# annihilatorrrr/spacedrive

Hardware: AMD Instinct MI355X
Metric: cas_ids/sec + hashed GB/s (whole node), 10M files at 1/2/4/8 MI355X (higher is better)
Workload: dtype u32; 1 GPU; sampled-path cas_id (57,352-B BLAKE3 message/file) + Object grouping; 1310720 files/GPU/step (1310720 per step at n_gpus=1); dup_permille=300, parallelism=shard-by-file x1, grouping=fused

## Files before the change

include/sd_hip_cas.h:

```cpp
#ifndef SD_HIP_CAS_H
#define SD_HIP_CAS_H

#include <stddef.h>
#include <stdint.h>

#ifdef __cplusplus
extern "C" {
#endif

#define SD_CAS_ABI_VERSION 1

#define SD_CAS_SAMPLE_COUNT 4u
#define SD_CAS_SAMPLE_SIZE (1024u * 10u)
#define SD_CAS_HEADER_OR_FOOTER_SIZE (1024u * 8u)
#define SD_CAS_MINIMUM_FILE_SIZE (1024u * 100u)
#define SD_CAS_SAMPLED_CONTENT_LEN (2u * SD_CAS_HEADER_OR_FOOTER_SIZE + SD_CAS_SAMPLE_COUNT * SD_CAS_SAMPLE_SIZE)
#define SD_CAS_CHUNK_SIZE 100u
#define SD_CAS_MAX_PACKED_CONTENT_LEN (104u * 1024u - 8u)

#define SD_CAS_OK 0
#define SD_CAS_EINVAL (-1)
#define SD_CAS_EHIP (-2)
#define SD_CAS_EIO (-3)
#define SD_CAS_ENOMEM (-4)
// ... 50 lines not shown
                               const char* prefix, uint32_t stride, char* d_out, void* stream);

int sd_cas_hash_sampled_dev(sd_cas_ctx* ctx, const void* d_content, uint64_t stride,
                            const uint64_t* d_sizes, size_t n, uint64_t* d_keys, void* stream);

int sd_cas_hash_packed_dev(sd_cas_ctx* ctx, const void* d_arena, const uint64_t* d_offs,
                           const uint32_t* d_lens, const uint64_t* d_sizes, size_t n,
                           uint64_t* d_keys, void* stream);

int sd_cas_group_dev(sd_cas_ctx* ctx, const uint64_t* d_keys, size_t n, uint32_t* d_rep,
                     uint64_t* out_objects, void* stream);
int sd_cas_hash_group_sampled_dev(sd_cas_ctx* ctx, const void* d_content, uint64_t stride,
                                  const uint64_t* d_sizes, size_t n, uint64_t* d_keys,
                                  uint32_t* d_rep, uint32_t* d_overflow, uint64_t* out_objects,
                                  void* stream);
int sd_cas_hash_regions_sampled_dev(sd_cas_ctx* ctx, const void* d_content, uint64_t stride,
                                    const uint64_t* d_sizes, size_t n, uint64_t* d_keys,
                                    uint32_t* d_rep, uint32_t* d_overflow, void* stream);
int sd_cas_group_regions_dev(sd_cas_ctx* ctx, size_t n, uint32_t* d_rep, uint64_t* out_objects,
                             void* stream);
int sd_cas_set_dup_verify(sd_cas_ctx* ctx, int on);
int sd_cas_dup_verify_counters(sd_cas_ctx* ctx, uint64_t* out_candidates, uint64_t* out_verified,
                               uint64_t* out_rehashed);
int sd_cas_group_min_dev(sd_cas_ctx* ctx, const uint64_t* d_keys, const uint32_t* d_vals, size_t n,
                         uint32_t* d_out, uint64_t* out_objects, void* stream);
int sd_cas_partition_dev(sd_cas_ctx* ctx, const uint64_t* d_keys, size_t n, uint32_t parts,
                         uint64_t* d_keys_out, uint32_t* d_pos_out, uint64_t* d_counts,
                         void* stream);
int sd_cas_exchange_pack_dev(sd_cas_ctx* ctx, const uint64_t* d_keys, const uint32_t* d_pos,
                             size_t n, uint64_t file0, uint32_t* d_rows, void* stream);
int sd_cas_exchange_split_dev(sd_cas_ctx* ctx, const uint32_t* d_rows, size_t m,
                              uint64_t* d_keys, uint32_t* d_vals, void* stream);
int sd_cas_exchange_unpack_dev(sd_cas_ctx* ctx, const uint32_t* d_back, const uint32_t* d_pos,
                               size_t n, uint64_t* d_rep, void* stream);
int sd_cas_exchange_pack_fixed_dev(sd_cas_ctx* ctx, const uint64_t* d_keys, const uint32_t* d_pos,
                                   const uint64_t* d_counts, uint32_t G, uint64_t cap,
                                   uint64_t spill, uint64_t file0, uint32_t* d_rows,
                                   uint32_t* d_spill_rows, uint32_t* d_overflow, void* stream);
int sd_cas_exchange_split_fixed_dev(sd_cas_ctx* ctx, const uint32_t* d_rows, size_t m,
                                    uint64_t sentinel, uint64_t* d_keys, uint32_t* d_vals,
                                    uint64_t* d_sentinel_rows, void* stream);
int sd_cas_exchange_unpack_fixed_dev(sd_cas_ctx* ctx, const uint32_t* d_back,
                                     const uint32_t* d_spill_back, const uint32_t* d_pos,
                                     const uint64_t* d_counts, uint32_t G, uint64_t cap,
                                     uint64_t spill, uint64_t* d_rep, void* stream);
int sd_cas_copy_objects_dev(sd_cas_ctx* ctx, uint64_t* d_dst, void* stream);
// ... 125 lines not shown
```

rust/sd-hip-cas/src/lib.rs:

```rust
#![allow(non_camel_case_types)]
use std::{
    ffi::{c_char, c_int, c_void, CStr, CString},
    io,
    os::unix::ffi::OsStrExt,
    path::{Path, PathBuf},
    ptr,
};

#[repr(C)]
pub struct sd_cas_ctx {
    _p: [u8; 0],
}

#[repr(C)]
pub struct sd_cas_multi {
    _p: [u8; 0],
}

pub const SD_CAS_ROW_HASHED: u8 = 0;
pub const SD_CAS_ROW_NO_CAS: u8 = 1;
pub const SD_CAS_ROW_ERROR: u8 = 2;
pub const SD_CAS_LINK_CREATED: u8 = 0;
pub const SD_CAS_LINK_LINKED: u8 = 1;
pub const SD_CAS_LINK_DROPPED: u8 = 2;
// ... 52 lines not shown
                                      prefix: *const c_char, stride: u32, d_out: *mut c_char,
                                      stream: *mut c_void) -> c_int;
    pub fn sd_cas_hash_sampled_dev(ctx: *mut sd_cas_ctx, d_content: *const c_void, stride: u64,
                                   d_sizes: *const u64, n: usize, d_keys: *mut u64,
                                   stream: *mut c_void) -> c_int;
    pub fn sd_cas_hash_packed_dev(ctx: *mut sd_cas_ctx, d_arena: *const c_void, d_offs: *const u64,
                                  d_lens: *const u32, d_sizes: *const u64, n: usize, d_keys: *mut u64,
                                  stream: *mut c_void) -> c_int;
    pub fn sd_cas_group_dev(ctx: *mut sd_cas_ctx, d_keys: *const u64, n: usize, d_rep: *mut u32,
                            out_objects: *mut u64, stream: *mut c_void) -> c_int;
    pub fn sd_cas_hash_group_sampled_dev(ctx: *mut sd_cas_ctx, d_content: *const c_void, stride: u64,
                                         d_sizes: *const u64, n: usize, d_keys: *mut u64,
                                         d_rep: *mut u32, d_overflow: *mut u32,
                                         out_objects: *mut u64, stream: *mut c_void) -> c_int;
    pub fn sd_cas_hash_regions_sampled_dev(ctx: *mut sd_cas_ctx, d_content: *const c_void, stride: u64,
                                           d_sizes: *const u64, n: usize, d_keys: *mut u64,
                                           d_rep: *mut u32, d_overflow: *mut u32,
                                           stream: *mut c_void) -> c_int;
    pub fn sd_cas_group_regions_dev(ctx: *mut sd_cas_ctx, n: usize, d_rep: *mut u32,
                                    out_objects: *mut u64, stream: *mut c_void) -> c_int;
    pub fn sd_cas_set_dup_verify(ctx: *mut sd_cas_ctx, on: c_int) -> c_int;
    pub fn sd_cas_dup_verify_counters(ctx: *mut sd_cas_ctx, out_candidates: *mut u64,
                                      out_verified: *mut u64, out_rehashed: *mut u64) -> c_int;
    pub fn sd_cas_group_min_dev(ctx: *mut sd_cas_ctx, d_keys: *const u64, d_vals: *const u32, n: usize,
                                d_out: *mut u32, out_objects: *mut u64, stream: *mut c_void) -> c_int;
    pub fn sd_cas_partition_dev(ctx: *mut sd_cas_ctx, d_keys: *const u64, n: usize, parts: u32,
                                d_keys_out: *mut u64, d_pos_out: *mut u32, d_counts: *mut u64,
                                stream: *mut c_void) -> c_int;
    pub fn sd_cas_exchange_pack_dev(ctx: *mut sd_cas_ctx, d_keys: *const u64, d_pos: *const u32,
                                    n: usize, file0: u64, d_rows: *mut u32, stream: *mut c_void) -> c_int;
    pub fn sd_cas_exchange_split_dev(ctx: *mut sd_cas_ctx, d_rows: *const u32, m: usize,
                                     d_keys: *mut u64, d_vals: *mut u32, stream: *mut c_void) -> c_int;
    pub fn sd_cas_exchange_unpack_dev(ctx: *mut sd_cas_ctx, d_back: *const u32, d_pos: *const u32,
                                      n: usize, d_rep: *mut u64, stream: *mut c_void) -> c_int;
    pub fn sd_cas_exchange_pack_fixed_dev(ctx: *mut sd_cas_ctx, d_keys: *const u64, d_pos: *const u32,
                                          d_counts: *const u64, G: u32, cap: u64, spill: u64,
                                          file0: u64, d_rows: *mut u32, d_spill_rows: *mut u32,
                                          d_overflow: *mut u32, stream: *mut c_void) -> c_int;
    pub fn sd_cas_exchange_split_fixed_dev(ctx: *mut sd_cas_ctx, d_rows: *const u32, m: usize,
                                           sentinel: u64, d_keys: *mut u64, d_vals: *mut u32,
                                           d_sentinel_rows: *mut u64, stream: *mut c_void) -> c_int;
    pub fn sd_cas_exchange_unpack_fixed_dev(ctx: *mut sd_cas_ctx, d_back: *const u32,
                                            d_spill_back: *const u32, d_pos: *const u32,
                                            d_counts: *const u64, G: u32, cap: u64, spill: u64,
                                            d_rep: *mut u64, stream: *mut c_void) -> c_int;
    pub fn sd_cas_copy_objects_dev(ctx: *mut sd_cas_ctx, d_dst: *mut u64, stream: *mut c_void) -> c_int;
// ... 508 lines not shown
```

spacedrive_amd/_native.py:

```python
from __future__ import annotations

import ctypes
import os
import subprocess

HERE = os.path.dirname(os.path.abspath(__file__))
LIB_PATH = os.environ.get("SD_HIP_CAS_LIB") or os.path.join(HERE, "libsd_hip_cas.so")
CSRC = os.path.join(HERE, "csrc")

SD_CAS_OK = 0
ERRORS = {-1: "EINVAL", -2: "EHIP", -3: "EIO", -4: "ENOMEM", -5: "ENODEV"}

_vp, _sz, _u64, _u32, _i = ctypes.c_void_p, ctypes.c_size_t, ctypes.c_uint64, ctypes.c_uint32, ctypes.c_int
_cp = ctypes.c_char_p
SIGNATURES = [
    ("sd_cas_abi_version", _i, []),
    ("sd_cas_ctx_create", _i, [_i, ctypes.POINTER(_vp)]),
    ("sd_cas_ctx_destroy", None, [_vp]),
    ("sd_cas_last_error", _cp, [_vp]),
    ("sd_cas_ctx_stream", _vp, [_vp]),
    ("sd_cas_synchronize", _i, [_vp]),
    ("sd_cas_batch_quantum", _sz, [_vp]),
    ("sd_cas_set_latency_threshold", None, [_vp, _sz, _sz]),
    ("sd_cas_set_chunkpar_split", None, [_vp, _sz, _sz]),
    ("sd_cas_set_group_method", _i, [_vp, _i, _u64]),
    ("sd_cas_alloc_pinned", _i, [_vp, _sz, ctypes.POINTER(_vp)]),
    ("sd_cas_free_pinned", _i, [_vp, _vp]),
    ("sd_cas_generate_cas_ids", _i, [_vp, _vp, _vp, _vp, _sz, _vp]),
    ("sd_cas_generate_cas_ids_from_paths", _i, [_vp, _vp, _vp, _sz, _vp, _vp]),
    ("sd_cas_file_metadata_from_paths", _i, [_vp, _vp, _sz, _vp, _vp, _vp]),
    ("sd_cas_hash_sampled_host", _i, [_vp, _vp, _u64, _vp, _sz, _vp, _sz]),
    ("sd_cas_hash_sampled_host_ring", _i, [_vp, _vp, _u64, _sz, _vp, _sz, _vp, _sz]),
    ("sd_cas_key_to_hex", None, [_u64, _cp]),
    ("sd_cas_shard_hex", None, [_u64, _cp]),
    ("sd_cas_thumbnail_path", ctypes.c_int64, [_cp, _cp, _u64, _cp, _sz]),
    ("sd_cas_thumb_key", ctypes.c_int64, [_cp, _u64, _cp, _sz]),
    ("sd_cas_keys_to_hex_dev", _i, [_vp, _vp, _sz, _vp, _vp]),
    ("sd_cas_thumbnail_paths_dev", _i, [_vp, _vp, _sz, _cp, _u32, _vp, _vp]),
    ("sd_cas_hash_sampled_dev", _i, [_vp, _vp, _u64, _vp, _sz, _vp, _vp]),
    ("sd_cas_hash_packed_dev", _i, [_vp, _vp, _vp, _vp, _vp, _sz, _vp, _vp]),
    ("sd_cas_group_dev", _i, [_vp, _vp, _sz, _vp, _vp, _vp]),
    ("sd_cas_hash_group_sampled_dev", _i, [_vp, _vp, _u64, _vp, _sz, _vp, _vp, _vp, _vp, _vp]),
    ("sd_cas_hash_regions_sampled_dev", _i, [_vp, _vp, _u64, _vp, _sz, _vp, _vp, _vp, _vp]),
    ("sd_cas_group_regions_dev", _i, [_vp, _sz, _vp, _vp, _vp]),
    ("sd_cas_set_dup_verify", _i, [_vp, _i]),
    ("sd_cas_dup_verify_counters", _i, [_vp, _vp, _vp, _vp]),
    ("sd_cas_group_min_dev", _i, [_vp, _vp, _vp, _sz, _vp, _vp, _vp]),
    ("sd_cas_partition_dev", _i, [_vp, _vp, _sz, _u32, _vp, _vp, _vp, _vp]),
    ("sd_cas_exchange_pack_dev", _i, [_vp, _vp, _vp, _sz, _u64, _vp, _vp]),
    ("sd_cas_exchange_split_dev", _i, [_vp, _vp, _sz, _vp, _vp, _vp]),
    ("sd_cas_exchange_unpack_dev", _i, [_vp, _vp, _vp, _sz, _vp, _vp]),
    ("sd_cas_exchange_pack_fixed_dev", _i, [_vp, _vp, _vp, _vp, _u32, _u64, _u64, _u64, _vp, _vp, _vp, _vp]),
    ("sd_cas_exchange_split_fixed_dev", _i, [_vp, _vp, _sz, _u64, _vp, _vp, _vp, _vp]),
    ("sd_cas_exchange_unpack_fixed_dev", _i, [_vp, _vp, _vp, _vp, _vp, _u32, _u64, _u64, _vp, _vp]),
    ("sd_cas_copy_objects_dev", _i, [_vp, _vp, _vp]),
    ("sd_cas_group_sorted_dev", _i, [_vp, _vp, _vp, _sz, _vp, _vp, _vp]),
    ("sd_cas_group_chunked_dev", _i, [_vp, _vp, _sz, _u32, _vp, _vp, _vp, _vp]),
    ("sd_cas_identifier_max_steps", _sz, [_sz, _u32]),
    ("sd_cas_identifier_links_dev", _i, [_vp, _vp, _vp, _sz, _u32, _vp, _vp, _vp, _vp, _sz, _vp, _vp]),
    ("sd_cas_identifier_links", _i, [_vp, _vp, _vp, _sz, _u32, _vp, _vp, _vp, _vp, _sz, _vp]),
    ("sd_cas_identifier_links_seeded_dev", _i,
     [_vp, _vp, _vp, _sz, _u32, _vp, _vp, _sz, _vp, _vp, _vp, _vp, _sz, _vp, _vp]),
    ("sd_cas_identifier_links_seeded", _i,
     [_vp, _vp, _vp, _sz, _u32, _vp, _vp, _sz, _vp, _vp, _vp, _vp, _sz, _vp]),
    ("sd_cas_identifier_links_ex_dev", _i,
     [_vp, _vp, _vp, _sz, _u32, _vp, _vp, _sz, _vp, _vp, _vp, _vp, _vp, _sz, _vp, _vp]),
    ("sd_cas_identifier_links_ex", _i,
     [_vp, _vp, _vp, _sz, _u32, _vp, _vp, _sz, _vp, _vp, _vp, _vp, _vp, _sz, _vp]),
    ("sd_cas_object_stats_dev", _i, [_vp, _vp, _vp, _sz, _vp, _vp, _vp, _vp]),
# ... 63 lines not shown
```

spacedrive_amd/cas.py:

```python
from __future__ import annotations

import ctypes
import os
from dataclasses import dataclass, field
from typing import Optional, Sequence

import numpy as np

from . import _native
from ._native import CasError

SAMPLE_COUNT = 4
SAMPLE_SIZE = 1024 * 10
HEADER_OR_FOOTER_SIZE = 1024 * 8
MINIMUM_FILE_SIZE = 1024 * 100
SAMPLED_CONTENT_LEN = 2 * HEADER_OR_FOOTER_SIZE + SAMPLE_COUNT * SAMPLE_SIZE
CHUNK_SIZE = 100
MAX_PACKED_CONTENT_LEN = 104 * 1024 - 8
THRESHOLD_DEFAULT = (1 << 64) - 1
NO_OBJECT = NO_STEP = 0xFFFFFFFF
STAT_NAMES = ("rows", "objects", "total_bytes", "unique_bytes", "duplicate_sets", "max_copies",
              "size_mismatch_rows", "bad_rows")
TOP_MAX = 65536
TOP_TILE = 16384
# ... 290 lines not shown
                             stream: Optional[int] = None) -> None:
        n = int(sizes.numel())
        stride = int(content.shape[-1]) if content.dim() == 2 else SAMPLED_CONTENT_LEN
        self._check(self.L.sd_cas_hash_regions_sampled_dev(
            self.h, _ptr(content), stride, _ptr(sizes), n, _ptr(keys), _ptr(rep), _ptr(overflow),
            _stream(stream)), "hash_regions_sampled")

    def group_regions(self, n: int, rep, stream: Optional[int] = None,
                      want_objects: bool = True) -> Optional[int]:
        obj = ctypes.c_uint64(0)
        self._check(self.L.sd_cas_group_regions_dev(self.h, int(n), _ptr(rep),
                                                    ctypes.byref(obj) if want_objects else None,
                                                    _stream(stream)), "group_regions")
        return int(obj.value) if want_objects else None

    def set_dup_verify(self, on: bool = True) -> None:
        self._check(self.L.sd_cas_set_dup_verify(self.h, 1 if on else 0), "set_dup_verify")

    def dup_verify_counters(self) -> tuple[int, int, int]:
        c, v, r = ctypes.c_uint64(0), ctypes.c_uint64(0), ctypes.c_uint64(0)
        self._check(self.L.sd_cas_dup_verify_counters(self.h, ctypes.byref(c), ctypes.byref(v),
                                                      ctypes.byref(r)), "dup_verify_counters")
        return int(c.value), int(v.value), int(r.value)

    def group_min(self, keys, vals, out, stream: Optional[int] = None,
                  want_objects: bool = True) -> Optional[int]:
        n = int(keys.numel())
        obj = ctypes.c_uint64(0)
        self._check(self.L.sd_cas_group_min_dev(
            self.h, _ptr(keys), _ptr(vals) if vals is not None else None, n, _ptr(out),
            ctypes.byref(obj) if want_objects else None, _stream(stream)), "group_min")
        return int(obj.value) if want_objects else None

    def exchange_pack(self, keys, pos, file0: int, rows, stream: Optional[int] = None) -> None:
        self._check(self.L.sd_cas_exchange_pack_dev(self.h, _ptr(keys), _ptr(pos), int(keys.numel()),
                                                    int(file0), _ptr(rows), _stream(stream)),
                    "exchange_pack")

    def exchange_split(self, rows, keys, vals, stream: Optional[int] = None) -> None:
        self._check(self.L.sd_cas_exchange_split_dev(self.h, _ptr(rows), int(keys.numel()), _ptr(keys),
                                                     _ptr(vals), _stream(stream)), "exchange_split")

    def exchange_unpack(self, back, pos, rep, stream: Optional[int] = None) -> None:
        self._check(self.L.sd_cas_exchange_unpack_dev(self.h, _ptr(back), _ptr(pos), int(back.numel()),
                                                      _ptr(rep), _stream(stream)), "exchange_unpack")

# ... 388 lines not shown
```

spacedrive_amd/csrc/cas_hash.hip:

```cpp
#include <hip/hip_runtime.h>
#include <stdint.h>

#include "blake3_lane.hpp"
#include "blake3_tree.hpp"
#include "sd_dup_probe.h"
#include "sd_group.h"
#include "sd_kernels.h"
#include "sd_mix.h"
#include "sd_ws.h"

namespace sdcas {


constexpr uint32_t SAMPLED_PAIRS = SAMPLED_CONTENT_LEN / 128;
constexpr uint32_t SAMPLED_CHUNKS = SAMPLED_CONTENT_LEN / 1024;
static_assert(SAMPLED_PAIRS == 8 * SAMPLED_CHUNKS, "the sampled content is whole chunks of 8 lines");

__device__ __forceinline__ void load_pair_here(const uint4* __restrict__ q, uint32_t P,
                                               uint4 (&buf)[8]) {
  __builtin_amdgcn_sched_barrier(0);
  line(q, P, buf);
  __builtin_amdgcn_sched_barrier(0);
}

constexpr int SAMPLED_DEPTH = 5;
constexpr int SAMPLED_BLOCK = 512;

template <int B = SAMPLED_BLOCK>
// ... 150 lines not shown
  if (blockIdx.x == 0 && threadIdx.x < 2) ro.objects[threadIdx.x] = 0;
  region_epilogue<B>(stack_lds, live, f, key, keys, ro);
}

extern "C" __global__ void __launch_bounds__(SAMPLED_BLOCK)
sd_cas_sampled_group_kernel(const uint8_t* __restrict__ content, uint64_t stride,
                            const uint64_t* __restrict__ sizes, uint64_t n,
                            uint64_t* __restrict__ keys, RegionOut ro) {
  sampled_group_kernel_body<SAMPLED_BLOCK>(content, stride, sizes, n, keys, ro);
}

extern "C" __global__ void __launch_bounds__(SAMPLED_BLOCK_NARROW)
sd_cas_sampled_group_kernel_256(const uint8_t* __restrict__ content, uint64_t stride,
                                const uint64_t* __restrict__ sizes, uint64_t n,
                                uint64_t* __restrict__ keys, RegionOut ro) {
  sampled_group_kernel_body<SAMPLED_BLOCK_NARROW>(content, stride, sizes, n, keys, ro);
}

struct DupLists {
  const uint32_t* cand;
  uint32_t* list_h;
  uint32_t* list_c;
  uint32_t* same;
  uint32_t* counters;
  uint32_t tail_tiles;
  volatile uint32_t* note;
  uint32_t seq, files;
};
constexpr uint32_t DUP_N_HASH = 0, DUP_N_CAND = 1, DUP_VERIFIED = 2, DUP_REHASHED = 3, DUP_QUEUE = 4;

extern "C" __global__ void __launch_bounds__(256)
sd_dup_probe_kernel(const uint8_t* __restrict__ content, uint64_t stride,
                    const uint64_t* __restrict__ sizes, uint64_t n, uint64_t* __restrict__ probes,
                    uint32_t* __restrict__ counters) {
  const uint64_t f = (uint64_t)blockIdx.x * 256 + threadIdx.x;
  if (blockIdx.x == 0 && threadIdx.x < DUP_COUNTERS) counters[threadIdx.x] = 0;
  if (f < n) probes[f] = dup_probe(sizes[f], content + f * stride);
}

extern "C" __global__ void __launch_bounds__(256)
sd_dup_compact_kernel(uint64_t n, DupLists dl) {
  __shared__ uint32_t wcnt[2][4], base[2];
  const uint64_t f = (uint64_t)blockIdx.x * 256 + threadIdx.x;
  const uint32_t lane = threadIdx.x & 63u, w = threadIdx.x >> 6;
  const bool live = f < n;
  const bool h = live && dl.cand[f] == (uint32_t)f;
  const bool c = live && !h;
  const uint64_t bh = __ballot(h), bc = __ballot(c);
  const uint64_t below = (1ull << lane) - 1ull;
  if (lane == 0) {
    wcnt[0][w] = (uint32_t)__popcll(bh);
    wcnt[1][w] = (uint32_t)__popcll(bc);
  }
  __syncthreads();
  if (threadIdx.x < 2) {
    const uint32_t t = wcnt[threadIdx.x][0] + wcnt[threadIdx.x][1] + wcnt[threadIdx.x][2] +
                       wcnt[threadIdx.x][3];
    base[threadIdx.x] = t ? atomicAdd(&dl.counters[threadIdx.x ? DUP_N_CAND : DUP_N_HASH], t) : 0u;
  }
  __syncthreads();
  uint32_t oh = base[0] + (uint32_t)__popcll(bh & below);
  uint32_t oc = base[1] + (uint32_t)__popcll(bc & below);
  for (uint32_t i = 0; i < w; ++i) {
    oh += wcnt[0][i];
    oc += wcnt[1][i];
  }
  if (h) dl.list_h[oh] = (uint32_t)f;
  if (c) dl.list_c[oc] = (uint32_t)f;
}

constexpr uint32_t CMP_QUADS = SAMPLED_CONTENT_LEN / 16;
constexpr uint32_t CMP_UNROLL = 8;
static_assert(CMP_QUADS % (64 * CMP_UNROLL) == 0, "a row is whole compare rounds");
__device__ __forceinline__ bool rows_equal(const uint4* __restrict__ a, const uint4* __restrict__ b,
                                           uint32_t lane) {
#pragma unroll 1
  for (uint32_t q = lane; q < CMP_QUADS; q += 64 * CMP_UNROLL) {
    uint4 x[CMP_UNROLL], y[CMP_UNROLL];
#pragma unroll
    for (uint32_t u = 0; u < CMP_UNROLL; ++u) x[u] = a[q + 64 * u];
#pragma unroll
    for (uint32_t u = 0; u < CMP_UNROLL; ++u) y[u] = b[q + 64 * u];
    uint32_t d = 0;
#pragma unroll
    for (uint32_t u = 0; u < CMP_UNROLL; ++u)
      d |= (x[u].x ^ y[u].x) | (x[u].y ^ y[u].y) | (x[u].z ^ y[u].z) | (x[u].w ^ y[u].w);
    if (__ballot(d != 0)) return false;
  }
  return true;
}

template <int B>
__device__ __forceinline__ void dup_mixed_kernel_body(const uint8_t* __restrict__ content,
                                                      uint64_t stride,
                                                      const uint64_t* __restrict__ sizes,
                                                      uint64_t* __restrict__ keys, RegionOut ro,
                                                      DupLists dl) {
  __shared__ uint32_t stack_lds[SAMPLED_DEPTH][8][B];
  const uint32_t n_hash = dl.counters[DUP_N_HASH], n_cand = dl.counters[DUP_N_CAND];
  const uint32_t G = gridDim.x;
  const uint32_t TH = (n_hash + B - 1) / B;
  const uint32_t TC = G - TH;
  const uint32_t TT = TC < dl.tail_tiles ? TC : dl.tail_tiles;
  const uint32_t GI = G - TT, TI = TC - TT;
  const bool tail = blockIdx.x >= GI;
  const uint32_t c0 = tail ? 0u : (uint32_t)((uint64_t)blockIdx.x * TI / GI);
  const uint32_t c1 = tail ? 1u : (uint32_t)(((uint64_t)blockIdx.x + 1) * TI / GI);
  if (blockIdx.x == 0 && threadIdx.x < 2) ro.objects[threadIdx.x] = 0;
  if (blockIdx.x == 0 && threadIdx.x == 0 && dl.note) {
    dl.note[1] = n_cand;
    dl.note[2] = dl.files;
    __threadfence_system();
    dl.note[0] = dl.seq;
  }
  if (c0 == c1) {
    const uint32_t i = (blockIdx.x - c0) * B + threadIdx.x;
    const bool live = i < n_hash;
    uint64_t f = 0, key = 0;
    if (live) {
      f = dl.list_h[i];
      LdsStack<B> stk{stack_lds, threadIdx.x};
      const uint4* q = reinterpret_cast<const uint4*>(content + f * stride);
      key = cas_lane_sampled<B>(q, sizes[f], stk);
    }
    region_epilogue<B>(stack_lds, live, f, key, keys, ro);
  } else {
    const uint32_t lane = threadIdx.x & 63u;
    for (uint32_t k = 0; tail || k < 64u; ++k) {
      uint32_t p = 0;
      if (lane == 0) p = atomicAdd(&dl.counters[DUP_QUEUE], 1u);
      p = __builtin_amdgcn_readfirstlane(p);
      if (p >= n_cand) break;
      const uint32_t f = dl.list_c[p], g = dl.cand[f];
      bool eq = sizes[f] == sizes[g];
      if (eq)
        eq = rows_equal(reinterpret_cast<const uint4*>(content + (uint64_t)f * stride),
                        reinterpret_cast<const uint4*>(content + (uint64_t)g * stride), lane);
      if (lane == 0) dl.same[f] = eq ? 1u : 0u;
    }
  }
}

extern "C" __global__ void __launch_bounds__(SAMPLED_BLOCK)
sd_cas_dup_mixed_kernel(const uint8_t* __restrict__ content, uint64_t stride,
                        const uint64_t* __restrict__ sizes, uint64_t* __restrict__ keys,
                        RegionOut ro, DupLists dl) {
  dup_mixed_kernel_body<SAMPLED_BLOCK>(content, stride, sizes, keys, ro, dl);
}

extern "C" __global__ void __launch_bounds__(SAMPLED_BLOCK_NARROW)
sd_cas_dup_mixed_kernel_256(const uint8_t* __restrict__ content, uint64_t stride,
                            const uint64_t* __restrict__ sizes, uint64_t* __restrict__ keys,
                            RegionOut ro, DupLists dl) {
  dup_mixed_kernel_body<SAMPLED_BLOCK_NARROW>(content, stride, sizes, keys, ro, dl);
}

extern "C" __global__ void __launch_bounds__(SAMPLED_BLOCK_NARROW)
sd_cas_dup_finish_kernel(const uint8_t* __restrict__ content, uint64_t stride,
                         const uint64_t* __restrict__ sizes, uint64_t* __restrict__ keys,
                         RegionOut ro, DupLists dl) {
  constexpr int B = SAMPLED_BLOCK_NARROW;
// ... 163 lines not shown
                                uint32_t* rfile, uint32_t* cursor, uint64_t cap, uint64_t* spill_keys,
                                uint32_t* spill_file, uint32_t* overflow, uint64_t* objects,
                                hipStream_t s, uint32_t cus) {
  if (n == 0) return hipSuccess;
  const RegionOut ro{rkeys, rfile, cursor, cap, spill_keys, spill_file, rep, overflow,
                     (unsigned long long*)objects};
  const uint64_t blocks = (n + SAMPLED_BLOCK - 1) / SAMPLED_BLOCK;
  const uint64_t quanta = cus ? (n + (uint64_t)cus * 256 - 1) / ((uint64_t)cus * 256) : 0;
  if (cus && (blocks < cus || (quanta & 1))) {
    const uint64_t nb = (n + SAMPLED_BLOCK_NARROW - 1) / SAMPLED_BLOCK_NARROW;
    sd_cas_sampled_group_kernel_256<<<(uint32_t)nb, SAMPLED_BLOCK_NARROW, 0, s>>>(content, stride,
                                                                                 sizes, n, keys, ro);
  } else {
    sd_cas_sampled_group_kernel<<<(uint32_t)blocks, SAMPLED_BLOCK, 0, s>>>(content, stride, sizes, n,
                                                                          keys, ro);
  }
  return hipGetLastError();
}

DupVerifyWs dup_verify_layout(void* ws, uint64_t n) {
  WsCarve w(ws);  DupVerifyWs L;
  L.probes = w.take<uint64_t>(n);  L.cand = w.take<uint32_t>(n);
  L.list_h = w.take<uint32_t>(n);  L.list_c = w.take<uint32_t>(n);  L.same = w.take<uint32_t>(n);
  L.counters = w.take<uint32_t>(DUP_COUNTERS);  L.objects = w.take<uint64_t>(1);
  L.bytes = w.bytes();  return L;
}
size_t dup_verify_workspace_bytes(uint64_t n) { return dup_verify_layout(nullptr, n).bytes; }

hipError_t dup_candidates(const uint8_t* content, uint64_t stride, const uint64_t* sizes, uint64_t n,
                          const DupVerifyWs& L, void* group_ws, uint32_t* totals, hipStream_t s) {
  if (n == 0) return hipSuccess;
  sd_dup_probe_kernel<<<(uint32_t)((n + 255) / 256), 256, 0, s>>>(content, stride, sizes, n, L.probes,
                                                                  L.counters);
  hipError_t e = hipGetLastError();
  if (e != hipSuccess) return e;
  return hash_group_min(L.probes, nullptr, n, L.cand, L.objects, group_ws, totals, s);
}

hipError_t hash_sampled_regions_verify(const uint8_t* content, uint64_t stride, const uint64_t* sizes,
                                       uint64_t n, uint64_t* keys, uint32_t* rep, uint64_t* rkeys,
                                       uint32_t* rfile, uint32_t* cursor, uint64_t cap,
                                       uint64_t* spill_keys, uint32_t* spill_file, uint32_t* overflow,
                                       uint64_t* objects, const DupVerifyWs& L, uint32_t* note,
                                       uint32_t seq, hipStream_t s, uint32_t cus) {
  if (n == 0) return hipSuccess;
  const RegionOut ro{rkeys, rfile, cursor, cap, spill_keys, spill_file, rep, overflow,
                     (unsigned long long*)objects};
  const uint64_t blocks = (n + SAMPLED_BLOCK - 1) / SAMPLED_BLOCK;
  const uint64_t quanta = cus ? (n + (uint64_t)cus * 256 - 1) / ((uint64_t)cus * 256) : 0;
  const bool narrow = cus && (blocks < cus || (quanta & 1));
  const uint32_t slots = (cus ? cus : 256u) * (narrow ? 4u : 2u);
  const uint32_t tail_tiles = slots * 5u / 7u;
  const DupLists dl{L.cand, L.list_h, L.list_c, L.same, L.counters, tail_tiles, note, seq, (uint32_t)n};
  sd_dup_compact_kernel<<<(uint32_t)((n + 255) / 256), 256, 0, s>>>(n, dl);
  if (narrow) {
    const uint64_t nb = (n + SAMPLED_BLOCK_NARROW - 1) / SAMPLED_BLOCK_NARROW;
    sd_cas_dup_mixed_kernel_256<<<(uint32_t)nb + 1, SAMPLED_BLOCK_NARROW, 0, s>>>(content, stride, sizes,
                                                                                 keys, ro, dl);
  } else {
    sd_cas_dup_mixed_kernel<<<(uint32_t)blocks + 1, SAMPLED_BLOCK, 0, s>>>(content, stride, sizes, keys,
                                                                          ro, dl);
  }
  const uint64_t fb = (n + SAMPLED_BLOCK_NARROW - 1) / SAMPLED_BLOCK_NARROW;
  sd_cas_dup_finish_kernel<<<(uint32_t)fb, SAMPLED_BLOCK_NARROW, 0, s>>>(content, stride, sizes, keys,
                                                                        ro, dl);
  return hipGetLastError();
}

#ifndef SD_PULL_UNROLL
#define SD_PULL_UNROLL 4
#endif
#ifndef SD_PULL_WIDE_BYTES
#define SD_PULL_WIDE_BYTES (512u << 10)
#endif
template <int U>
__global__ void __launch_bounds__(256)
sd_pull_host(const uint4* __restrict__ src, uint4* __restrict__ dst, uint64_t quads) {
// ... 59 lines not shown
```

spacedrive_amd/csrc/sd_hip_cas.cpp:

```cpp
#include <ctype.h>
#include <errno.h>
#include <fcntl.h>
#include <hip/hip_runtime.h>
#include <stdarg.h>
#include <stdio.h>
#include <stdlib.h>
#include <string.h>
#include <sys/stat.h>
#include <unistd.h>

#include <algorithm>
#include <atomic>
#include <memory>
#include <string>
#include <thread>
#include <vector>

#include "sd_checksum.h"
#include "sd_group.h"
#include "sd_kernels.h"
#include "sd_links.h"
#include "sd_mix.h"
#include "sd_object_stats.h"
#include "sd_synth.h"
// ... 527 lines not shown
      e = hash_sampled_regions_verify((const uint8_t*)d_content, stride, d_sizes, n, d_keys, d_rep,
                                      L.rkeys, L.rfile, cur, region_capacity(n), L.spill_keys,
                                      L.spill_file, d_overflow, L.objects, D, c->dupv_note,
                                      ++c->dupv_seq, s, (uint32_t)(c->quantum / 256));
    c->dupv_n = e == hipSuccess ? n : 0;
    c->dupv_stream = s;
  } else {
    e = hash_sampled_regions((const uint8_t*)d_content, stride, d_sizes, n, d_keys, d_rep,
                             L.rkeys, L.rfile, cur, region_capacity(n), L.spill_keys,
                             L.spill_file, d_overflow, L.objects, s, (uint32_t)(c->quantum / 256));
    c->dupv_n = 0;
  }
  if (e != hipSuccess) {
    (void)hipMemsetAsync(cur, 0, REGION_SET_WORDS * 4, s);
    return fail(c, SD_CAS_EHIP, "hash_regions: %s", hipGetErrorString(e));
  }
  HIP_TRY(c, hipEventRecord(c->region_hashed[k], s));
  c->region_keys[k] = d_keys;
  c->region_cur = k;
  c->region_grouped[k] = false;
  return SD_CAS_OK;
}

int sd_cas_dup_verify_counters(sd_cas_ctx* c, uint64_t* out_candidates, uint64_t* out_verified,
                               uint64_t* out_rehashed) {
  if (!c || !out_candidates || !out_verified || !out_rehashed) return SD_CAS_EINVAL;
  uint32_t h[DUP_COUNTERS] = {0};
  if (c->dupv_n && c->region_cur >= 0) {
    HIP_TRY(c, hipSetDevice(c->device));
    HIP_TRY(c, hipStreamWaitEvent(c->stream, c->region_hashed[c->region_cur], 0));
    HIP_TRY(c, hipMemcpyAsync(h, dup_verify_layout(c->dupv.p, c->dupv_n).counters, sizeof h,
                              hipMemcpyDeviceToHost, c->stream));
    HIP_TRY(c, hipStreamSynchronize(c->stream));
  }
  *out_candidates = h[1];
  *out_verified = h[2];
  *out_rehashed = h[3];
  return SD_CAS_OK;
}

int sd_cas_group_regions_dev(sd_cas_ctx* c, size_t n, uint32_t* d_rep, uint64_t* out_objects,
                             void* stream) {
  if (!c) return SD_CAS_EINVAL;
  const int k = c->region_cur;
  if (k < 0 || c->region_grouped[k] || c->region_n[k] != n || !d_rep)
    return fail(c, SD_CAS_EINVAL, "group_regions: no ungrouped hash_regions batch of %zu files", n);
  HIP_TRY(c, hipSetDevice(c->device));
  hipStream_t s = pick(c, stream);
  const RegionGroupWs L = region_group_layout(c->regions[k].p, c->region_n[k]);
  uint32_t* cur = c->gcursor + REGION_SET_WORDS * k;
  HIP_TRY(c, hipStreamWaitEvent(s, c->region_hashed[k], 0));
  hipError_t e = region_group_min(L.rkeys, L.rfile, cur, region_capacity(n), d_rep, L.objects, L.gkeys, L.gvals,
                                  c->region_keys[k], n, L.spill_keys, L.spill_file, c->test_table_fill, s);
  if (e != hipSuccess) {
    (void)hipMemsetAsync(cur, 0, REGION_SET_WORDS * 4, s);
    return fail(c, SD_CAS_EHIP, "group_regions: %s", hipGetErrorString(e));
  }
  HIP_TRY(c, hipEventRecord(c->region_done[k], s));
  c->region_pending[k] = true;
  c->region_grouped[k] = true;
// ... 590 lines not shown
```

spacedrive_amd/csrc/sd_kernels.h:

```cpp
#pragma once
#include <stdint.h>

namespace sdcas {

constexpr uint64_t SAMPLE_COUNT = 4;
constexpr uint64_t SAMPLE_SIZE = 1024 * 10;
constexpr uint64_t HEADER_OR_FOOTER_SIZE = 1024 * 8;
constexpr uint64_t MINIMUM_FILE_SIZE = 1024 * 100;
constexpr uint32_t SAMPLED_CONTENT_LEN =
    (uint32_t)(2 * HEADER_OR_FOOTER_SIZE + SAMPLE_COUNT * SAMPLE_SIZE);
static_assert(2 * HEADER_OR_FOOTER_SIZE + SAMPLE_COUNT * SAMPLE_SIZE < MINIMUM_FILE_SIZE, "cas.rs:18");
static_assert(SAMPLE_SIZE > HEADER_OR_FOOTER_SIZE, "cas.rs:21");

constexpr uint32_t MAX_PACKED_CONTENT_LEN = 104u * 1024u - 8u;

}

#include <hip/hip_runtime.h>
namespace sdcas {
hipError_t hash_sampled(const uint8_t* content, uint64_t stride, const uint64_t* sizes,
                        uint64_t n, uint64_t* keys, hipStream_t s, uint32_t cus);
hipError_t hash_sampled_regions(const uint8_t* content, uint64_t stride, const uint64_t* sizes,
                                uint64_t n, uint64_t* keys, uint32_t* rep, uint64_t* rkeys,
                                uint32_t* rfile, uint32_t* cursor, uint64_t cap, uint64_t* spill_keys,
                                uint32_t* spill_file, uint32_t* overflow, uint64_t* objects,
                                hipStream_t s, uint32_t cus);
constexpr uint32_t DUP_COUNTERS = 8;
struct DupVerifyWs {
  uint64_t* probes; uint32_t *cand, *list_h, *list_c, *same, *counters; uint64_t* objects; size_t bytes;
};
DupVerifyWs dup_verify_layout(void* ws, uint64_t n);
size_t dup_verify_workspace_bytes(uint64_t n);
hipError_t dup_candidates(const uint8_t* content, uint64_t stride, const uint64_t* sizes, uint64_t n,
                          const DupVerifyWs& L, void* group_ws, uint32_t* totals, hipStream_t s);
hipError_t hash_sampled_regions_verify(const uint8_t* content, uint64_t stride, const uint64_t* sizes,
                                       uint64_t n, uint64_t* keys, uint32_t* rep, uint64_t* rkeys,
                                       uint32_t* rfile, uint32_t* cursor, uint64_t cap,
                                       uint64_t* spill_keys, uint32_t* spill_file, uint32_t* overflow,
                                       uint64_t* objects, const DupVerifyWs& L, uint32_t* note,
                                       uint32_t seq, hipStream_t s, uint32_t cus);
hipError_t pull_host(void* dst, const void* src, uint64_t bytes, hipStream_t s);
hipError_t hash_packed(const uint8_t* arena, const uint64_t* offs, const uint32_t* lens,
                       const uint64_t* sizes, const uint32_t* order, uint64_t n, uint64_t* keys,
                       hipStream_t s);
hipError_t length_keys(const uint32_t* lens, uint64_t n, uint64_t* out, hipStream_t s);
hipError_t hash_chunkpar(const uint8_t* arena, const uint64_t* offs, uint64_t stride,
                         const uint32_t* lens, uint32_t fixed_len, const uint64_t* sizes,
                         uint64_t n, uint64_t* keys, int seg, hipStream_t s,
                         const uint32_t* order = nullptr);
int length_key_bits(uint64_t n);
struct InplaceWs { uint32_t *counters, *lens32, *sampled_idx; size_t bytes; };
InplaceWs inplace_layout(void* ws, uint64_t n);
// ... 8 lines not shown
```

Baseline: 60.72 million cas_ids/s.

## Batch duplicate verification into grouped runs sharing reference slice loads

After: 61.62 million cas_ids/s (median of 6 runs). 1.5% higher.

```diff
diff --git a/include/sd_hip_cas.h b/include/sd_hip_cas.h
--- a/include/sd_hip_cas.h
+++ b/include/sd_hip_cas.h
@@ -96,6 +96,8 @@
 int sd_cas_set_dup_verify(sd_cas_ctx* ctx, int on);
 int sd_cas_dup_verify_counters(sd_cas_ctx* ctx, uint64_t* out_candidates, uint64_t* out_verified,
                                uint64_t* out_rehashed);
+int sd_cas_dup_verify_rows(sd_cas_ctx* ctx, uint64_t* out_groups, uint64_t* out_tasks,
+                           uint64_t* out_references);
 int sd_cas_group_min_dev(sd_cas_ctx* ctx, const uint64_t* d_keys, const uint32_t* d_vals, size_t n,
                          uint32_t* d_out, uint64_t* out_objects, void* stream);
 int sd_cas_partition_dev(sd_cas_ctx* ctx, const uint64_t* d_keys, size_t n, uint32_t parts,
diff --git a/rust/sd-hip-cas/src/lib.rs b/rust/sd-hip-cas/src/lib.rs
--- a/rust/sd-hip-cas/src/lib.rs
+++ b/rust/sd-hip-cas/src/lib.rs
@@ -98,6 +98,8 @@
     pub fn sd_cas_set_dup_verify(ctx: *mut sd_cas_ctx, on: c_int) -> c_int;
     pub fn sd_cas_dup_verify_counters(ctx: *mut sd_cas_ctx, out_candidates: *mut u64,
                                       out_verified: *mut u64, out_rehashed: *mut u64) -> c_int;
+    pub fn sd_cas_dup_verify_rows(ctx: *mut sd_cas_ctx, out_groups: *mut u64, out_tasks: *mut u64,
+                                  out_references: *mut u64) -> c_int;
     pub fn sd_cas_group_min_dev(ctx: *mut sd_cas_ctx, d_keys: *const u64, d_vals: *const u32, n: usize,
                                 d_out: *mut u32, out_objects: *mut u64, stream: *mut c_void) -> c_int;
     pub fn sd_cas_partition_dev(ctx: *mut sd_cas_ctx, d_keys: *const u64, n: usize, parts: u32,
diff --git a/spacedrive_amd/_native.py b/spacedrive_amd/_native.py
--- a/spacedrive_amd/_native.py
+++ b/spacedrive_amd/_native.py
@@ -45,6 +45,7 @@
     ("sd_cas_group_regions_dev", _i, [_vp, _sz, _vp, _vp, _vp]),
     ("sd_cas_set_dup_verify", _i, [_vp, _i]),
     ("sd_cas_dup_verify_counters", _i, [_vp, _vp, _vp, _vp]),
+    ("sd_cas_dup_verify_rows", _i, [_vp, _vp, _vp, _vp]),
     ("sd_cas_group_min_dev", _i, [_vp, _vp, _vp, _sz, _vp, _vp, _vp]),
     ("sd_cas_partition_dev", _i, [_vp, _vp, _sz, _u32, _vp, _vp, _vp, _vp]),
     ("sd_cas_exchange_pack_dev", _i, [_vp, _vp, _vp, _sz, _u64, _vp, _vp]),
diff --git a/spacedrive_amd/cas.py b/spacedrive_amd/cas.py
--- a/spacedrive_amd/cas.py
+++ b/spacedrive_amd/cas.py
@@ -336,6 +336,12 @@
         self._check(self.L.sd_cas_dup_verify_counters(self.h, ctypes.byref(c), ctypes.byref(v),
                                                       ctypes.byref(r)), "dup_verify_counters")
         return int(c.value), int(v.value), int(r.value)
+
+    def dup_verify_rows(self) -> tuple[int, int, int]:
+        g, t, r = ctypes.c_uint64(0), ctypes.c_uint64(0), ctypes.c_uint64(0)
+        self._check(self.L.sd_cas_dup_verify_rows(self.h, ctypes.byref(g), ctypes.byref(t),
+                                                  ctypes.byref(r)), "dup_verify_rows")
+        return int(g.value), int(t.value), int(r.value)
 
     def group_min(self, keys, vals, out, stream: Optional[int] = None,
                   want_objects: bool = True) -> Optional[int]:
diff --git a/spacedrive_amd/csrc/cas_hash.hip b/spacedrive_amd/csrc/cas_hash.hip
--- a/spacedrive_amd/csrc/cas_hash.hip
+++ b/spacedrive_amd/csrc/cas_hash.hip
@@ -4,6 +4,7 @@
 #include "blake3_lane.hpp"
 #include "blake3_tree.hpp"
 #include "sd_dup_probe.h"
+#include "sd_dup_runs.h"
 #include "sd_group.h"
 #include "sd_kernels.h"
 #include "sd_mix.h"
@@ -200,72 +201,155 @@
   uint32_t* list_h;
   uint32_t* list_c;
   uint32_t* same;
+  uint32_t* cnt;
+  uint32_t* first;
+  uint32_t* rank;
   uint32_t* counters;
   uint32_t tail_tiles;
   volatile uint32_t* note;
   uint32_t seq, files;
 };
-constexpr uint32_t DUP_N_HASH = 0, DUP_N_CAND = 1, DUP_VERIFIED = 2, DUP_REHASHED = 3, DUP_QUEUE = 4;
+constexpr uint32_t DUP_N_HASH = 0, DUP_N_CAND = 1, DUP_VERIFIED = 2, DUP_REHASHED = 3, DUP_QUEUE = 4,
+                   DUP_GROUPS = 5, DUP_TASKS = 6, DUP_REFS = 7;
+static_assert(DUP_REFS < DUP_COUNTERS, "counters");
 
 extern "C" __global__ void __launch_bounds__(256)
 sd_dup_probe_kernel(const uint8_t* __restrict__ content, uint64_t stride,
                     const uint64_t* __restrict__ sizes, uint64_t n, uint64_t* __restrict__ probes,
-                    uint32_t* __restrict__ counters) {
+                    uint32_t* __restrict__ counters, uint32_t* __restrict__ cnt) {
   const uint64_t f = (uint64_t)blockIdx.x * 256 + threadIdx.x;
   if (blockIdx.x == 0 && threadIdx.x < DUP_COUNTERS) counters[threadIdx.x] = 0;
-  if (f < n) probes[f] = dup_probe(sizes[f], content + f * stride);
+  if (f < n) {
+    probes[f] = dup_probe(sizes[f], content + f * stride);
+    cnt[f] = 0;
+  }
 }
 
 extern "C" __global__ void __launch_bounds__(256)
 sd_dup_compact_kernel(uint64_t n, DupLists dl) {
-  __shared__ uint32_t wcnt[2][4], base[2];
+  __shared__ uint32_t wcnt[3][4], base;
   const uint64_t f = (uint64_t)blockIdx.x * 256 + threadIdx.x;
   const uint32_t lane = threadIdx.x & 63u, w = threadIdx.x >> 6;
   const bool live = f < n;
-  const bool h = live && dl.cand[f] == (uint32_t)f;
+  const uint32_t g = live ? dl.cand[f] : 0u;
+  const bool h = live && g == (uint32_t)f;
   const bool c = live && !h;
-  const uint64_t bh = __ballot(h), bc = __ballot(c);
+  uint32_t r = 1;
+  if (c) {
+    r = atomicAdd(&dl.cnt[g], 1u);
+    dl.rank[f] = r;
+  }
+  const uint64_t bh = __ballot(h), bc = __ballot(c), bg = __ballot(r == 0);
   const uint64_t below = (1ull << lane) - 1ull;
   if (lane == 0) {
     wcnt[0][w] = (uint32_t)__popcll(bh);
     wcnt[1][w] = (uint32_t)__popcll(bc);
+    wcnt[2][w] = (uint32_t)__popcll(bg);
   }
   __syncthreads();
-  if (threadIdx.x < 2) {
+  if (threadIdx.x < 3) {
+    constexpr uint32_t word[3] = {DUP_N_HASH, DUP_N_CAND, DUP_GROUPS};
     const uint32_t t = wcnt[threadIdx.x][0] + wcnt[threadIdx.x][1] + wcnt[threadIdx.x][2] +
                        wcnt[threadIdx.x][3];
-    base[threadIdx.x] = t ? atomicAdd(&dl.counters[threadIdx.x ? DUP_N_CAND : DUP_N_HASH], t) : 0u;
+    const uint32_t b = t ? atomicAdd(&dl.counters[word[threadIdx.x]], t) : 0u;
+    if (threadIdx.x == 0) base = b;
   }
   __syncthreads();
-  uint32_t oh = base[0] + (uint32_t)__popcll(bh & below);
-  uint32_t oc = base[1] + (uint32_t)__popcll(bc & below);
-  for (uint32_t i = 0; i < w; ++i) {
-    oh += wcnt[0][i];
-    oc += wcnt[1][i];
-  }
+  uint32_t oh = base + (uint32_t)__popcll(bh & below);
+  for (uint32_t i = 0; i < w; ++i) oh += wcnt[0][i];
   if (h) dl.list_h[oh] = (uint32_t)f;
-  if (c) dl.list_c[oc] = (uint32_t)f;
-}
-
-constexpr uint32_t CMP_QUADS = SAMPLED_CONTENT_LEN / 16;
-constexpr uint32_t CMP_UNROLL = 8;
-static_assert(CMP_QUADS % (64 * CMP_UNROLL) == 0, "a row is whole compare rounds");
-__device__ __forceinline__ bool rows_equal(const uint4* __restrict__ a, const uint4* __restrict__ b,
-                                           uint32_t lane) {
+}
+
+extern "C" __global__ void __launch_bounds__(256)
+sd_dup_order_kernel(uint64_t n, DupLists dl) {
+  const uint64_t f = (uint64_t)blockIdx.x * 256 + threadIdx.x;
+  if (f >= n) return;
+  const uint32_t g = dl.cand[f];
+  if (g != (uint32_t)f) dl.list_c[dl.first[g] + dl.rank[f]] = (uint32_t)f;
+}
+
+struct DupSlice { uint4 q[DUP_SLICE_QUADS]; };
+typedef uint32_t dup_u32x4 __attribute__((ext_vector_type(4)));
+__device__ __forceinline__ void dup_load_slice(DupSlice& d, const uint8_t* __restrict__ content,
+                                               uint64_t stride, uint32_t file, uint32_t s, uint32_t voff) {
+  const uint64_t a = (uint64_t)content + (uint64_t)file * stride;
+  const uint64_t row = ((uint64_t)(uint32_t)__builtin_amdgcn_readfirstlane((int)(a >> 32)) << 32) |
+                       (uint32_t)__builtin_amdgcn_readfirstlane((int)(uint32_t)a);
+  const __amdgpu_buffer_rsrc_t rsrc =
+      __builtin_amdgcn_make_buffer_rsrc((void*)row, 0, (int)DUP_ROW_BYTES, 0x00020000);
+#pragma unroll
+  for (uint32_t u = 0; u < DUP_SLICE_QUADS; ++u) {
+    const dup_u32x4 v = __builtin_amdgcn_raw_buffer_load_b128(rsrc, (int)voff,
+                                                              (int)dup_slice_quad_offset(s, u, 0), 0);
+    d.q[u] = make_uint4(v.x, v.y, v.z, v.w);
+  }
+}
+__device__ __forceinline__ bool dup_slices_differ(const DupSlice& a, const DupSlice& b) {
+  uint32_t d = 0;
+#pragma unroll
+  for (uint32_t u = 0; u < DUP_SLICE_QUADS; ++u)
+    d |= (a.q[u].x ^ b.q[u].x) | (a.q[u].y ^ b.q[u].y) | (a.q[u].z ^ b.q[u].z) | (a.q[u].w ^ b.q[u].w);
+  return __builtin_amdgcn_ballot_w64(d != 0) != 0;
+}
+__device__ __forceinline__ uint32_t dup_lane_of(uint32_t voff) {
+  uint32_t lane;
+  asm volatile("v_lshrrev_b32 %0, 4, %1" : "=v"(lane) : "v"(voff));
+  return lane;
+}
+__device__ __forceinline__ uint32_t dup_first_bit(uint32_t m) {
+  return (uint32_t)__builtin_amdgcn_readfirstlane(__builtin_ctz(m));
+}
+
+__device__ __forceinline__ uint32_t dup_compare_task(const uint8_t* __restrict__ content, uint64_t stride,
+                                                     const uint64_t* __restrict__ sizes,
+                                                     const DupLists& dl, uint32_t t, uint32_t n_cand,
+                                                     uint32_t voff) {
+  uint32_t lane = dup_lane_of(voff);
+  const uint32_t first = dup_task_first(t), m = dup_task_entries(t, n_cand);
+  uint32_t f = 0, g = 0;
+  bool ok = false;
+  if (lane < m) {
+    f = dl.list_c[first + lane];
+    g = dl.cand[f];
+    ok = sizes[f] == sizes[g];
+  }
+  bool head = lane < m;
+  if (head && lane) head = dl.first[g] == first + lane;
+  const uint32_t heads = (uint32_t)__ballot(head);
+  const uint32_t runs = (uint32_t)__builtin_popcount(heads);
+  uint32_t alive = (uint32_t)__ballot(ok);
 #pragma unroll 1
-  for (uint32_t q = lane; q < CMP_QUADS; q += 64 * CMP_UNROLL) {
-    uint4 x[CMP_UNROLL], y[CMP_UNROLL];
-#pragma unroll
-    for (uint32_t u = 0; u < CMP_UNROLL; ++u) x[u] = a[q + 64 * u];
-#pragma unroll
-    for (uint32_t u = 0; u < CMP_UNROLL; ++u) y[u] = b[q + 64 * u];
-    uint32_t d = 0;
-#pragma unroll
-    for (uint32_t u = 0; u < CMP_UNROLL; ++u)
-      d |= (x[u].x ^ y[u].x) | (x[u].y ^ y[u].y) | (x[u].z ^ y[u].z) | (x[u].w ^ y[u].w);
-    if (__ballot(d != 0)) return false;
-  }
-  return true;
+  for (uint32_t s = 0; s < DUP_SLICES && alive; ++s) {
+    DupSlice ref, cur, nxt;
+    uint32_t left = alive;
+    uint32_t e = dup_first_bit(left);
+    uint32_t fe = (uint32_t)__builtin_amdgcn_readlane((int)f, (int)e);
+    uint32_t loaded = (uint32_t)__builtin_popcount(heads & ((2u << e) - 1u));
+    dup_load_slice(ref, content, stride, (uint32_t)__builtin_amdgcn_readfirstlane((int)dl.cand[fe]), s, voff);
+    dup_load_slice(cur, content, stride, fe, s, voff);
+#pragma unroll 1
+    for (;;) {
+      left &= left - 1u;
+      uint32_t e2 = 0;
+      if (left) {
+        e2 = dup_first_bit(left);
+        fe = (uint32_t)__builtin_amdgcn_readlane((int)f, (int)e2);
+        dup_load_slice(nxt, content, stride, fe, s, voff);
+      }
+      if (dup_slices_differ(ref, cur)) alive &= ~(1u << e);
+      if (!left) break;
+      e = e2;
+      cur = nxt;
+      const uint32_t run = (uint32_t)__builtin_popcount(heads & ((2u << e) - 1u));
+      if (run != loaded) {
+        loaded = run;
+        dup_load_slice(ref, content, stride, (uint32_t)__builtin_amdgcn_readfirstlane((int)dl.cand[fe]), s, voff);
+      }
+    }
+  }
+  lane = dup_lane_of(voff);
+  if (lane < m) dl.same[f] = (alive >> lane) & 1u;
+  return runs;
 }
 
 template <int B>
@@ -278,12 +362,7 @@
   const uint32_t n_hash = dl.counters[DUP_N_HASH], n_cand = dl.counters[DUP_N_CAND];
   const uint32_t G = gridDim.x;
   const uint32_t TH = (n_hash + B - 1) / B;
-  const uint32_t TC = G - TH;
-  const uint32_t TT = TC < dl.tail_tiles ? TC : dl.tail_tiles;
-  const uint32_t GI = G - TT, TI = TC - TT;
-  const bool tail = blockIdx.x >= GI;
-  const uint32_t c0 = tail ? 0u : (uint32_t)((uint64_t)blockIdx.x * TI / GI);
-  const uint32_t c1 = tail ? 1u : (uint32_t)(((uint64_t)blockIdx.x + 1) * TI / GI);
+  const DupTile tile = dup_tile_of(blockIdx.x, G, TH, dl.tail_tiles);
   if (blockIdx.x == 0 && threadIdx.x < 2) ro.objects[threadIdx.x] = 0;
   if (blockIdx.x == 0 && threadIdx.x == 0 && dl.note) {
     dl.note[1] = n_cand;
@@ -291,8 +370,8 @@
     __threadfence_system();
     dl.note[0] = dl.seq;
   }
-  if (c0 == c1) {
-    const uint32_t i = (blockIdx.x - c0) * B + threadIdx.x;
+  if (!tile.compare) {
+    const uint32_t i = tile.hash_tile * B + threadIdx.x;
     const bool live = i < n_hash;
     uint64_t f = 0, key = 0;
     if (live) {
@@ -303,18 +382,20 @@
     }
     region_epilogue<B>(stack_lds, live, f, key, keys, ro);
   } else {
-    const uint32_t lane = threadIdx.x & 63u;
-    for (uint32_t k = 0; tail || k < 64u; ++k) {
-      uint32_t p = 0;
-      if (lane == 0) p = atomicAdd(&dl.counters[DUP_QUEUE], 1u);
-      p = __builtin_amdgcn_readfirstlane(p);
-      if (p >= n_cand) break;
-      const uint32_t f = dl.list_c[p], g = dl.cand[f];
-      bool eq = sizes[f] == sizes[g];
-      if (eq)
-        eq = rows_equal(reinterpret_cast<const uint4*>(content + (uint64_t)f * stride),
-                        reinterpret_cast<const uint4*>(content + (uint64_t)g * stride), lane);
-      if (lane == 0) dl.same[f] = eq ? 1u : 0u;
+    const uint32_t voff = dup_slice_quad_offset(0, 0, threadIdx.x & 63u);
+    const uint32_t n_tasks = dup_task_count(n_cand);
+    uint32_t done = 0, refs = 0;
+    for (uint32_t k = 0; tile.tail || k < dup_tile_wave_tasks(); ++k) {
+      uint32_t t = 0;
+      if (voff == 0) t = atomicAdd(&dl.counters[DUP_QUEUE], 1u);
+      t = __builtin_amdgcn_readfirstlane(t);
+      if (t >= n_tasks) break;
+      refs += dup_compare_task(content, stride, sizes, dl, t, n_cand, voff);
+      ++done;
+    }
+    if (voff == 0 && done) {
+      atomicAdd(&dl.counters[DUP_TASKS], done);
+      atomicAdd(&dl.counters[DUP_REFS], refs);
     }
   }
 }
@@ -524,16 +605,23 @@
   WsCarve w(ws);  DupVerifyWs L;
   L.probes = w.take<uint64_t>(n);  L.cand = w.take<uint32_t>(n);
   L.list_h = w.take<uint32_t>(n);  L.list_c = w.take<uint32_t>(n);  L.same = w.take<uint32_t>(n);
+  L.cnt = w.take<uint32_t>(n);  L.first = w.take<uint32_t>(n);  L.rank = w.take<uint32_t>(n);
+  L.partial = w.take<uint32_t>(n / 4096 + 1);
   L.counters = w.take<uint32_t>(DUP_COUNTERS);  L.objects = w.take<uint64_t>(1);
   L.bytes = w.bytes();  return L;
 }
 size_t dup_verify_workspace_bytes(uint64_t n) { return dup_verify_layout(nullptr, n).bytes; }
+
+#ifndef SD_DUP_TAIL_NUM
+#define SD_DUP_TAIL_NUM 5u
+#define SD_DUP_TAIL_DEN 7u
+#endif
 
 hipError_t dup_candidates(const uint8_t* content, uint64_t stride, const uint64_t* sizes, uint64_t n,
                           const DupVerifyWs& L, void* group_ws, uint32_t* totals, hipStream_t s) {
   if (n == 0) return hipSuccess;
   sd_dup_probe_kernel<<<(uint32_t)((n + 255) / 256), 256, 0, s>>>(content, stride, sizes, n, L.probes,
-                                                                  L.counters);
+                                                                  L.counters, L.cnt);
   hipError_t e = hipGetLastError();
   if (e != hipSuccess) return e;
   return hash_group_min(L.probes, nullptr, n, L.cand, L.objects, group_ws, totals, s);
@@ -552,9 +640,14 @@
   const uint64_t quanta = cus ? (n + (uint64_t)cus * 256 - 1) / ((uint64_t)cus * 256) : 0;
   const bool narrow = cus && (blocks < cus || (quanta & 1));
   const uint32_t slots = (cus ? cus : 256u) * (narrow ? 4u : 2u);
-  const uint32_t tail_tiles = slots * 5u / 7u;
-  const DupLists dl{L.cand, L.list_h, L.list_c, L.same, L.counters, tail_tiles, note, seq, (uint32_t)n};
-  sd_dup_compact_kernel<<<(uint32_t)((n + 255) / 256), 256, 0, s>>>(n, dl);
+  const uint32_t tail_tiles = slots * SD_DUP_TAIL_NUM / SD_DUP_TAIL_DEN;
+  const DupLists dl{L.cand, L.list_h, L.list_c, L.same, L.cnt, L.first, L.rank, L.counters,
+                    tail_tiles, note, seq, (uint32_t)n};
+  const uint32_t nb256 = (uint32_t)((n + 255) / 256);
+  sd_dup_compact_kernel<<<nb256, 256, 0, s>>>(n, dl);
+  hipError_t e = exclusive_scan_u32(L.cnt, L.first, n, L.partial, s);
+  if (e != hipSuccess) return e;
+  sd_dup_order_kernel<<<nb256, 256, 0, s>>>(n, dl);
   if (narrow) {
     const uint64_t nb = (n + SAMPLED_BLOCK_NARROW - 1) / SAMPLED_BLOCK_NARROW;
     sd_cas_dup_mixed_kernel_256<<<(uint32_t)nb + 1, SAMPLED_BLOCK_NARROW, 0, s>>>(content, stride, sizes,
diff --git a/spacedrive_amd/csrc/sd_dup_runs.h b/spacedrive_amd/csrc/sd_dup_runs.h
--- /dev/null
+++ b/spacedrive_amd/csrc/sd_dup_runs.h
@@ -0,0 +1,53 @@
+#pragma once
+#include <stdint.h>
+
+#if defined(__HIPCC__)
+#define SD_RUNS_HD __host__ __device__
+#else
+#define SD_RUNS_HD
+#endif
+
+namespace sdcas {
+
+#ifndef SD_DUP_RUN_K
+#define SD_DUP_RUN_K 16
+#endif
+constexpr uint32_t DUP_RUN_K = SD_DUP_RUN_K;
+static_assert(DUP_RUN_K >= 1 && DUP_RUN_K <= 32, "a task's entries are the bits of one u32");
+
+constexpr uint32_t DUP_ROW_BYTES = 57344;
+constexpr uint32_t DUP_WAVE = 64;
+constexpr uint32_t DUP_SLICE_QUADS = 8;
+constexpr uint32_t DUP_SLICE_BYTES = DUP_WAVE * DUP_SLICE_QUADS * 16;
+constexpr uint32_t DUP_SLICES = DUP_ROW_BYTES / DUP_SLICE_BYTES;
+static_assert(DUP_SLICES * DUP_SLICE_BYTES == DUP_ROW_BYTES, "a row is whole slices");
+
+SD_RUNS_HD inline uint32_t dup_task_count(uint32_t n_cand) {
+  return n_cand / DUP_RUN_K + (n_cand % DUP_RUN_K ? 1u : 0u);
+}
+SD_RUNS_HD inline uint32_t dup_task_first(uint32_t t) { return t * DUP_RUN_K; }
+SD_RUNS_HD inline uint32_t dup_task_entries(uint32_t t, uint32_t n_cand) {
+  const uint32_t left = n_cand - dup_task_first(t);
+  return left < DUP_RUN_K ? left : DUP_RUN_K;
+}
+
+struct DupTile {
+  bool compare, tail;
+  uint32_t hash_tile;
+};
+SD_RUNS_HD inline DupTile dup_tile_of(uint32_t b, uint32_t G, uint32_t TH, uint32_t tail_tiles) {
+  const uint32_t TC = G - TH;
+  const uint32_t TT = TC < tail_tiles ? TC : tail_tiles;
+  const uint32_t GI = G - TT, TI = TC - TT;
+  if (b >= GI) return {true, true, 0u};
+  const uint32_t c0 = (uint32_t)((uint64_t)b * TI / GI);
+  const uint32_t c1 = (uint32_t)(((uint64_t)b + 1) * TI / GI);
+  return {c0 != c1, false, b - c0};
+}
+SD_RUNS_HD inline uint32_t dup_tile_wave_tasks(void) { return (DUP_WAVE + DUP_RUN_K - 1) / DUP_RUN_K; }
+
+SD_RUNS_HD inline uint32_t dup_slice_quad_offset(uint32_t s, uint32_t u, uint32_t lane) {
+  return s * DUP_SLICE_BYTES + (u * DUP_WAVE + lane) * 16u;
+}
+
+}
diff --git a/spacedrive_amd/csrc/sd_hip_cas.cpp b/spacedrive_amd/csrc/sd_hip_cas.cpp
--- a/spacedrive_amd/csrc/sd_hip_cas.cpp
+++ b/spacedrive_amd/csrc/sd_hip_cas.cpp
@@ -573,10 +573,7 @@
   return SD_CAS_OK;
 }
 
-int sd_cas_dup_verify_counters(sd_cas_ctx* c, uint64_t* out_candidates, uint64_t* out_verified,
-                               uint64_t* out_rehashed) {
-  if (!c || !out_candidates || !out_verified || !out_rehashed) return SD_CAS_EINVAL;
-  uint32_t h[DUP_COUNTERS] = {0};
+static int dup_verify_words(sd_cas_ctx* c, uint32_t (&h)[DUP_COUNTERS]) {
   if (c->dupv_n && c->region_cur >= 0) {
     HIP_TRY(c, hipSetDevice(c->device));
     HIP_TRY(c, hipStreamWaitEvent(c->stream, c->region_hashed[c->region_cur], 0));
@@ -584,9 +581,30 @@
                               hipMemcpyDeviceToHost, c->stream));
     HIP_TRY(c, hipStreamSynchronize(c->stream));
   }
+  return SD_CAS_OK;
+}
+
+int sd_cas_dup_verify_counters(sd_cas_ctx* c, uint64_t* out_candidates, uint64_t* out_verified,
+                               uint64_t* out_rehashed) {
+  if (!c || !out_candidates || !out_verified || !out_rehashed) return SD_CAS_EINVAL;
+  uint32_t h[DUP_COUNTERS] = {0};
+  const int rc = dup_verify_words(c, h);
+  if (rc) return rc;
   *out_candidates = h[1];
   *out_verified = h[2];
   *out_rehashed = h[3];
+  return SD_CAS_OK;
+}
+
+int sd_cas_dup_verify_rows(sd_cas_ctx* c, uint64_t* out_groups, uint64_t* out_tasks,
+                           uint64_t* out_references) {
+  if (!c || !out_groups || !out_tasks || !out_references) return SD_CAS_EINVAL;
+  uint32_t h[DUP_COUNTERS] = {0};
+  const int rc = dup_verify_words(c, h);
+  if (rc) return rc;
+  *out_groups = h[5];
+  *out_tasks = h[6];
+  *out_references = h[7];
   return SD_CAS_OK;
 }
 
diff --git a/spacedrive_amd/csrc/sd_kernels.h b/spacedrive_amd/csrc/sd_kernels.h
--- a/spacedrive_amd/csrc/sd_kernels.h
+++ b/spacedrive_amd/csrc/sd_kernels.h
@@ -27,7 +27,8 @@
                                 hipStream_t s, uint32_t cus);
 constexpr uint32_t DUP_COUNTERS = 8;
 struct DupVerifyWs {
-  uint64_t* probes; uint32_t *cand, *list_h, *list_c, *same, *counters; uint64_t* objects; size_t bytes;
+  uint64_t* probes; uint32_t *cand, *list_h, *list_c, *same, *cnt, *first, *rank, *partial, *counters;
+  uint64_t* objects; size_t bytes;
 };
 DupVerifyWs dup_verify_layout(void* ws, uint64_t n);
 size_t dup_verify_workspace_bytes(uint64_t n);
```
